# johanDDC/R-TuckER

Hardware: NVIDIA B200
Metric: train triples/s (1-N fwd+bwd+RSGD step), WN18RR (higher is better)
Workload: dtype f32 (score GEMMs and N x r x r passes: 3xTF32 on tcgen05 with round-to-nearest partial sums = fp32 accuracy, 1e-5 parity; Grams and N-independent stage f64)

## Files before the change

### r-tucker_b200/csrc/small.cu

```cuda
#include "small_kernels.cuh"
#include "small_exec.cuh"

#include <algorithm>
#include <vector>

namespace {
using namespace rt::small;
using rt::align_up;
using rt::cdiv;

constexpr int kNumT = 8;
constexpr int kMinDotSlots = 2048;
constexpr size_t kPartialArenaBytes = (size_t)592 * 64 * 64 * sizeof(double);

struct Layout {
  int r[3];
  int B;
  int64_t c;
  size_t C64, Gm[3], Ainv[3], coresq, Tn[kNumT], KC[3], Nn[3], Vf[3], GL[3], GLinv[3], Gs[3],
      tmpM[3], tmpK[3], sub[3], sub_shared, exec_bar, gemm_partial, gram_ws, dot_partial, scal, total;
  int dot_slots;
};

Layout make_layout(int r0, int r1, int r2, int B) {
// ... 253 lines not shown
           bool square_dev = false) {
    ew(EW_CVT, x, tx, n * dsize(tx), nullptr, 0, y, ty, n * dsize(ty), n, a_host, a_dev, 0.0, nullptr, square_dev ? 1 : 0);
  }
  void to32plain(const double* x, float* y, int64_t n) { cvt(x, DT_F64, y, DT_F32, n); }
  void scale32(const float* x, float* y, int64_t n, double a_host, const double* a_dev) { cvt(x, DT_F32, y, DT_F32, n, a_host, a_dev); }
  void to64(const float* x, double* y, int64_t n) { cvt(x, DT_F32, y, DT_F64, n); }
  void axpby(const double* x, const double* y, double* z, int64_t n, double a, const double* a_dev,
             double b, const double* b_dev) {
    ew(EW_AXPBY64, x, DT_F64, n * 8, y, n * 8, z, DT_F64, n * 8, n, a, a_dev, b, b_dev);
  }
  void copy2d(const void* src, int ts, int64_t lds, void* dst, int td, int64_t ldd, int rows, int cols) {
    ew(EW_CVT_2D, src, ts, ((size_t)(rows - 1) * lds + cols) * dsize(ts), nullptr, 0, dst, td,
       ((size_t)(rows - 1) * ldd + cols) * dsize(td), (int64_t)rows * cols, 1.0, nullptr, 0.0, nullptr, lds, ldd, rows, cols);
  }
  void transpose_into(const double* src, int n, double* dst, int64_t ldd) {
    ew(EW_TRANSPOSE_INTO, src, DT_F64, (size_t)n * n * 8, nullptr, 0, dst, DT_F64, ((size_t)(n - 1) * ldd + n) * 8,
       (int64_t)n * n, 1.0, nullptr, 0.0, nullptr, n, ldd, n, 0);
  }
  void symmetrize_lower(double* A, int n) {
    ew(EW_SYMM_LOWER, nullptr, DT_F64, 0, nullptr, 0, A, DT_F64, (size_t)n * n * 8, (int64_t)n * n, 1.0, nullptr, 0.0,
       nullptr, n, 0, n, 0, true);
  }
  void norm_finish(const double* sq, const double* hyper, double* norm_out, double* alpha_out) {
    if (err) return;
    Rec rec{};
    rec.op.kind = OP_EW; rec.op.ew = EW_NORM_FINISH; rec.op.units = 1;
    EwPart& e = rec.op.e;
    e.x = sq; e.y = alpha_out; e.z = norm_out; e.d0 = hyper; e.count = 1;
    rec.rd[rec.nrd++] = range(sq, 8);
    rec.rd[rec.nrd++] = range(hyper, 32);
    rec.wr[rec.nwr++] = range(norm_out, 8);
    rec.wr[rec.nwr++] = range(alpha_out, 8);
    push(rec);
  }
  void adam_finish(const double* sq, double* hyper, double* adam, double* norm_out, double* alpha_out) {
    if (err) return;
    Rec rec{};
    rec.op.kind = OP_EW; rec.op.ew = EW_ADAM_FINISH; rec.op.units = 1;
    EwPart& e = rec.op.e;
    e.x = sq; e.y = alpha_out; e.z = norm_out; e.d0 = hyper; e.d1 = adam; e.count = 1;
    rec.rd[rec.nrd++] = range(sq, 8);
    rec.rd[rec.nrd++] = range(adam, 64);
    rec.wr[rec.nwr++] = range(norm_out, 8);
    rec.wr[rec.nwr++] = range(alpha_out, 8);
    push(rec);
  }
  void zero64(double* z, int64_t n) { ew(EW_ZERO64, nullptr, DT_F64, 0, nullptr, 0, z, DT_F64, n * 8, n, 0.0, nullptr, 0.0, nullptr); }

  void dot(const void* x, int tx, const void* y, int ty, int64_t n, double scale, double* out, int accumulate) {
    if (err || n <= 0) return;
    const int64_t units64 = (n + kEwChunk - 1) / kEwChunk;
    if (units64 > L.dot_slots) {
      rt::set_error("small stage: a dot over %lld elements needs %lld partial slots, the workspace has %d",
                    (long long)n, (long long)units64, L.dot_slots);
      err = 2; return;
    }
    const int units = (int)units64;
    if (dot_off + units > L.dot_slots) { flush(); }
    double* part = p(L.dot_partial) + dot_off;
    dot_off += units;
    Rec rec{};
    rec.op.kind = OP_DOT;
    EwPart& e = rec.op.e;
    e.x = x; e.y = y; e.z = part; e.tx = tx; e.tz = ty; e.count = n;
    rec.op.units = units;
    rec.rd[rec.nrd++] = range(x, n * dsize(tx));
    rec.rd[rec.nrd++] = range(y, n * dsize(ty));
    rec.wr[rec.nwr++] = range(part, (size_t)units * 8);
    push(rec);
    Rec fin{};
    fin.op.kind = OP_DOTFIN;
    EwPart& f = fin.op.e;
    f.x = part; f.z = out; f.count = units; f.s0 = scale; f.p0 = accumulate;
    fin.op.units = 1;
    fin.rd[fin.nrd++] = range(part, (size_t)units * 8);
    if (accumulate) fin.rd[fin.nrd++] = range(out, 8);
    fin.wr[fin.nwr++] = range(out, 8);
    push(fin);
  }

  int spd(const SpdBatch& b, int count, int nmax) {
    flush();
    if (err) return 1;
    size_t smem = ((size_t)nmax * (nmax + 1) / 2 + (size_t)SPD_NB * nmax) * sizeof(double);
    const size_t smem_limit = 227 * 1024 - 3072;
    if (smem > smem_limit || nmax > 256) {
      rt::set_error("small stage: rank %d exceeds the in-shared-memory Cholesky limit (230)", nmax); return 2; }
    SpdBatch bb = b;
    bb.dmma = (smem + (size_t)SPD_NB * nmax * sizeof(double) <= smem_limit) ? 1 : 0;
    if (bb.dmma) smem += (size_t)SPD_NB * nmax * sizeof(double);
    if (cudaFuncSetAttribute(spd_blocked_kernel, cudaFuncAttributeMaxDynamicSharedMemorySize, (int)smem) != cudaSuccess) {
      rt::set_error("small stage: cannot raise shared memory to %zu", smem); return 1; }
    spd_blocked_kernel<<<count, SPD_THREADS, smem, s>>>(bb); ++rt::g_launches;
    return 0;
  }
};

int finish(Ctx& c, const char* what) {
  c.flush();
  if (c.err) { if (c.err == 1) rt::set_error("%s: kernel launch failed", what); return 1; }
  cudaError_t e = cudaGetLastError();
  if (e != cudaSuccess) { rt::set_error("%s: %s", what, cudaGetErrorString(e)); return 1; }
  return 0;
}

template <typename T>
void grouped_contract(Ctx& c, const T* X, const T* const B[3], const T* const Wa[3],
                      const T* const Wb[3], const int64_t st_o[3], const int64_t st_i[3],
                      T* D, T* E1, T* E2, T* U1, T* U2, T* out) {
  const int d[3] = {c.r(0), c.r(1), c.r(2)};
  c.mode_prod(0, Wa[0], st_o[0], st_i[0], d[0], d[0], X, d, D, 1.0, 0.0);
  c.mode_prod(0, Wb[0], st_o[0], st_i[0], d[0], d[0], B[0], d, D, 1.0, 1.0);
  c.mode_prod(0, Wa[0], st_o[0], st_i[0], d[0], d[0], B[1], d, E1, 1.0, 0.0);
  if (E2 != E1) c.mode_prod(0, Wa[0], st_o[0], st_i[0], d[0], d[0], B[2], d, E2, 1.0, 0.0);
  c.mode_prod(1, Wa[1], st_o[1], st_i[1], d[1], d[1], D, d, U1, 1.0, 0.0);
  c.mode_prod(1, Wb[1], st_o[1], st_i[1], d[1], d[1], E1, d, U1, 1.0, 1.0);
  c.mode_prod(1, Wa[1], st_o[1], st_i[1], d[1], d[1], E2, d, U2, 1.0, 0.0);
  c.mode_prod(2, Wa[2], st_o[2], st_i[2], d[2], d[2], U1, d, out, 1.0, 0.0);
  c.mode_prod(2, Wb[2], st_o[2], st_i[2], d[2], d[2], U2, d, out, 1.0, 1.0);
}

}

extern "C" size_t rt_small_ws_bytes(int r0, int r1, int r2, int B) {
  if (r0 <= 0 || r1 <= 0 || r2 <= 0) return 0;
  return make_layout(r0, r1, r2, B).total;
}

extern "C" int rt_small_prepare(const float* core, int r0, int r1, int r2, int sym, void* small_ws,
                                void* stream) {
  RT_REQUIRE(small_ws != nullptr && r0 > 0 && r1 > 0 && r2 > 0, "rt_small_prepare: bad arguments");
  RT_REQUIRE(!sym || r1 == r2, "rt_small_prepare: SF-Tucker needs r1 == r2");
  Ctx c{make_layout(r0, r1, r2, 0), (char*)small_ws, (cudaStream_t)stream};
  double* C64 = c.p(c.L.C64);
  c.to64(core, C64, c.L.c);
  const int d[3] = {r0, r1, r2};
  for (int i = 0; i < 3; ++i) c.unfold_gram(i, C64, d, C64, d[i], c.p(c.L.Gm[i]), d[i], 1.0, 0.0);
  if (sym) {
    c.axpby(c.p(c.L.Gm[1]), c.p(c.L.Gm[2]), c.p(c.L.Gm[1]), (int64_t)r1 * r1, 1.0, nullptr, 1.0, nullptr);
    c.axpby(c.p(c.L.Gm[1]), nullptr, c.p(c.L.Gm[2]), (int64_t)r1 * r1, 1.0, nullptr, 0.0, nullptr);
  }
  SpdBatch b{};
  int nmax = 0;
  for (int i = 0; i < 3; ++i) {
    b.p[i].G = c.p(c.L.Gm[i]); b.p[i].L = nullptr; b.p[i].Linv = nullptr; b.p[i].Ginv = c.p(c.L.Ainv[i]);
    b.p[i].n = d[i];
    nmax = d[i] > nmax ? d[i] : nmax;
  }
  c.dot(C64, DT_F64, C64, DT_F64, c.L.c, 1.0, c.p(c.L.coresq), 0);
  int rc = c.spd(b, 3, nmax);
  if (rc) return rc;
  return finish(c, "rt_small_prepare");
}

extern "C" size_t rt_small_ainv_offset(int mode, int r0, int r1, int r2) {
  if (mode < 0 || mode > 2) return (size_t)-1;
  return make_layout(r0, r1, r2, 0).Ainv[mode];
}

extern "C" int rt_rows_times_ainv(const float* A, int m, int mode, int r0, int r1, int r2, float* C,
                                  void* small_ws, void* stream) {
  RT_REQUIRE(mode >= 0 && mode < 3 && m >= 0, "rt_rows_times_ainv: bad arguments");
  if (m == 0) return 0;
  Layout L = make_layout(r0, r1, r2, 0);
  const int r = L.r[mode];
  const double* K = (const double*)((char*)small_ws + L.Ainv[mode]);
  const size_t smem = (size_t)4 * r * sizeof(float);
  rows_times_mat_kernel<<<cdiv(m, 4), 256, smem, (cudaStream_t)stream>>>(A, m, r, K, C);
  RT_LAUNCH_CHECK();
  return 0;
}

extern "C" int rt_small_grad(const float* core, const float* d_core, const float* qp, const float* H,
                             const float* r_rows, const float* s_rows, const float* dr_rows,
                             const float* ds_rows, const double* bce_sum, double inv_count,
                             const double* hyper, int B, int r0, int r1, int r2, int sym, float* dS_g,
// ... 211 lines not shown
```

### r-tucker_b200/csrc/small_kernels.cuh

```cuda
#pragma once
#include "common.h"
#include <math.h>

namespace rt {
namespace small {

__global__ void __launch_bounds__(256)
rows_times_mat_kernel(const float* __restrict__ A, int m, int r, const double* __restrict__ K,
                      float* __restrict__ C) {
  extern __shared__ float rows[];
  constexpr int RPB = 4;
  const int b0 = blockIdx.x * RPB;
  for (int e = threadIdx.x; e < RPB * r; e += 256) {
    const int rr = e / r, cc = e - rr * r;
    rows[e] = (b0 + rr < m) ? A[(int64_t)(b0 + rr) * r + cc] : 0.0f;
  }
  __syncthreads();
  for (int j = threadIdx.x; j < r; j += 256) {
    double acc[RPB];
#pragma unroll
    for (int i = 0; i < RPB; ++i) acc[i] = 0.0;
#pragma unroll 4
    for (int k = 0; k < r; ++k) {
      const double kv = K[(int64_t)k * r + j];
#pragma unroll
      for (int i = 0; i < RPB; ++i) acc[i] = fma((double)rows[i * r + k], kv, acc[i]);
    }
#pragma unroll
    for (int i = 0; i < RPB; ++i)
      if (b0 + i < m) C[(int64_t)(b0 + i) * r + j] = (float)acc[i];
  }
}

struct SpdProblem {
  const double* G;
  double* L;
  double* Linv;
  double* Ginv;
  int n;
};
struct SpdBatch { SpdProblem p[3]; int dmma; };

__device__ __forceinline__ int pk(int i, int j) { return i * (i + 1) / 2 + j; }
__device__ __forceinline__ void spd_dmma(double& c0, double& c1, double a, double b) {
  asm volatile("mma.sync.aligned.m8n8k4.row.col.f64.f64.f64.f64 {%0, %1}, {%2}, {%3}, {%0, %1};\n"
               : "+d"(c0), "+d"(c1) : "d"(a), "d"(b));
}
__device__ __forceinline__ double spd_sum8(const double (&c)[8][2], int e) {
  return ((c[0][e] + c[1][e]) + (c[2][e] + c[3][e])) + ((c[4][e] + c[5][e]) + (c[6][e] + c[7][e]));
}

constexpr int SPD_NB = 8;
constexpr int SPD_THREADS = 512, SPD_TPR = 2;
__global__ void __launch_bounds__(SPD_THREADS, 1)
spd_blocked_kernel(SpdBatch batch) {
  extern __shared__ double sm[];
  const SpdProblem P = batch.p[blockIdx.x];
  const int n = P.n;
  if (n <= 0) return;
  double* Lp = sm;
  double* stage = sm + n * (n + 1) / 2;
  __shared__ double D[SPD_NB][SPD_NB + 1], invd[SPD_NB];
  __shared__ double dinv_all[256];
  __shared__ double s_maxd, s_scale[4];
  const int tid = threadIdx.x, nt = blockDim.x;
  const int row = tid / SPD_TPR, sub = tid % SPD_TPR;
  for (int e = tid; e < n * (n + 1) / 2; e += nt) {
    int i = (int)((sqrt(8.0 * e + 1.0) - 1.0) * 0.5);
    while (i * (i + 1) / 2 > e) --i;
    while ((i + 1) * (i + 2) / 2 <= e) ++i;
    const int j = e - i * (i + 1) / 2;
    Lp[e] = 0.5 * (P.G[(int64_t)i * n + j] + P.G[(int64_t)j * n + i]);
  }
  __syncthreads();
  if (tid < 32) {
    double m = 0.0;
    for (int i = tid; i < n; i += 32) m = fmax(m, Lp[pk(i, i)]);
#pragma unroll
    for (int o = 16; o > 0; o >>= 1) m = fmax(m, __shfl_xor_sync(0xffffffffu, m, o));
    if (tid == 0) {
      int ex = 0;
      if (m > 0.0) { frexp(m, &ex); ex += ex & 1; }
      s_maxd = ldexp(m, -ex);
      s_scale[0] = ldexp(1.0, -ex);
      s_scale[1] = ldexp(1.0, ex / 2);
      s_scale[2] = ldexp(1.0, -(ex / 2));
      s_scale[3] = ldexp(1.0, -ex);
    }
  }
  __syncthreads();
  {
    const double sc = s_scale[0];
    for (int e = tid; e < n * (n + 1) / 2; e += nt) Lp[e] *= sc;
  }
  __syncthreads();
  const double tol = 1e-12 * s_maxd;
  double* Li = Lp + pk(row < n ? row : 0, 0);
#ifdef RT_SPD_PROF
  long long t_0 = clock64(), t_a = 0, t_b = 0, t_c = 0, t_x;
#define SPD_LAP(v) do { t_x = clock64(); v += t_x - t_0; t_0 = t_x; } while (0)
#else
#define SPD_LAP(v) do {} while (0)
#endif
  const bool use_dmma = batch.dmma != 0;
  const int warp = tid >> 5, lane = tid & 31, fg = lane >> 2, ft = lane & 3;
  constexpr int NW = SPD_THREADS / 32;
  double* accS = stage + SPD_NB * n;
  for (int kb = 0; kb < n; kb += SPD_NB) {
    const int nbk = min(SPD_NB, n - kb);
    if (use_dmma) {
      if (kb > 0) {
        const int ntile = (n - kb + 7) >> 3, nsteps = kb >> 2;
        const int brow = kb + fg;
        const bool bv = brow < n;
        const double* Lb = Lp + pk(bv ? brow : 0, 0) + ft;
        for (int tile = warp; tile < ntile; tile += NW) {
          const int arow = kb + 8 * tile + fg;
          const bool av = arow < n;
          const double* La = Lp + pk(av ? arow : 0, 0) + ft;
          double c[8][2];
#pragma unroll
          for (int u = 0; u < 8; ++u) { c[u][0] = 0.0; c[u][1] = 0.0; }
          for (int s0 = 0; s0 < nsteps; s0 += 8) {
#pragma unroll
            for (int u = 0; u < 8; ++u)
              if (s0 + u < nsteps) spd_dmma(c[u][0], c[u][1], av ? La[4 * (s0 + u)] : 0.0, bv ? Lb[4 * (s0 + u)] : 0.0);
          }
#pragma unroll
          for (int e = 0; e < 2; ++e) {
            const int col = 2 * ft + e;
            if (av && col < nbk && kb + col <= arow) Lp[pk(arow, kb + col)] -= spd_sum8(c, e);
          }
        }
      }
    } else {
      double acc[SPD_NB];
#pragma unroll
      for (int c = 0; c < SPD_NB; ++c) acc[c] = 0.0;
      if (row < n && row >= kb) {
        const double* Lc[SPD_NB];
#pragma unroll
        for (int c = 0; c < SPD_NB; ++c) Lc[c] = Lp + pk(kb + (c < nbk ? c : 0), 0);
        for (int k = sub; k < kb; k += SPD_TPR) {
          const double li = Li[k];
#pragma unroll
          for (int c = 0; c < SPD_NB; ++c) acc[c] = fma(li, Lc[c][k], acc[c]);
        }
      }
#pragma unroll
      for (int c = 0; c < SPD_NB; ++c) {
#pragma unroll
        for (int o = 1; o < SPD_TPR; o <<= 1) acc[c] += __shfl_xor_sync(0xffffffffu, acc[c], o);
      }
      if (row < n && row >= kb && sub == 0) {
#pragma unroll
        for (int c = 0; c < SPD_NB; ++c)
          if (c < nbk && kb + c <= row) Li[kb + c] -= acc[c];
      }
    }
    __syncthreads();
    SPD_LAP(t_a);
    if (tid < 32) {
      int er[2], ec[2];
#pragma unroll
      for (int u = 0; u < 2; ++u) {
        const int e = tid + 32 * u;
        int r = 0;
        while ((r + 1) * (r + 2) / 2 <= e) ++r;
        er[u] = r; ec[u] = e - r * (r + 1) / 2;
      }
      const bool has2 = tid + 32 < SPD_NB * (SPD_NB + 1) / 2;
      if (!has2) { er[1] = 0; ec[1] = 0; }
#pragma unroll
      for (int u = 0; u < 2; ++u)
        if (u == 0 || has2)
          D[er[u]][ec[u]] = (er[u] < nbk) ? Lp[pk(kb + er[u], kb + ec[u])] : (er[u] == ec[u] ? 1.0 : 0.0);
      __syncwarp();
#pragma unroll
      for (int c = 0; c < SPD_NB - 1; ++c) {
        const double dc = D[c][c];
        double a_rc[2], a_cc[2];
#pragma unroll
        for (int u = 0; u < 2; ++u) { a_rc[u] = D[er[u]][c]; a_cc[u] = D[ec[u]][c]; }
        double ri = 0.0;
        if (dc > tol) {
          double y = (double)__frcp_rn((float)dc);
          y = fma(y, fma(-dc, y, 1.0), y);
          ri = fma(y, fma(-dc, y, 1.0), y);
        }
#pragma unroll
        for (int u = 0; u < 2; ++u)
          if ((u == 0 || has2) && ec[u] > c) D[er[u]][ec[u]] = fma(-(a_rc[u] * a_cc[u]), ri, D[er[u]][ec[u]]);
        __syncwarp();
      }
      {
        const int c = tid & (SPD_NB - 1);
        const double dc = D[c][c];
        double piv = 0.0, inv = 0.0;
        if (dc > tol) {
          double y = (double)rsqrtf((float)dc);
#pragma unroll
          for (int it = 0; it < 2; ++it) y = y * fma(-0.5 * dc, y * y, 1.5);
          piv = dc * y;
          piv = fma(0.5 * y, fma(-piv, piv, dc), piv);
          inv = fma(y, fma(-piv, y, 1.0), y);
        }
        __syncwarp();
        if (tid < SPD_NB) {
          invd[c] = inv;
          if (c < nbk) dinv_all[kb + c] = inv;
        }
        __syncwarp();
#pragma unroll
        for (int u = 0; u < 2; ++u)
          if ((u == 0 || has2) && er[u] != ec[u]) D[er[u]][ec[u]] *= invd[ec[u]];
        if (tid < SPD_NB) D[c][c] = piv;
        __syncwarp();
#pragma unroll
        for (int u = 0; u < 2; ++u)
          if ((u == 0 || has2) && er[u] < nbk) Lp[pk(kb + er[u], kb + ec[u])] = D[er[u]][ec[u]];
      }
    }
    __syncthreads();
    SPD_LAP(t_b);
    if (row < n && row >= kb + nbk && sub == 0) {
      double xs[SPD_NB];
#pragma unroll
      for (int c = 0; c < SPD_NB; ++c) {
        if (c < nbk) {
          double x = Li[kb + c];
#pragma unroll
          for (int c2 = 0; c2 < SPD_NB; ++c2)
            if (c2 < c) x = fma(-xs[c2], D[c][c2], x);
          x *= invd[c];
          xs[c] = x;
          Li[kb + c] = x;
        }
      }
    }
    __syncthreads();
    SPD_LAP(t_c);
  }
#ifdef RT_SPD_PROF
  if (tid == 0) printf("spd n=%d chol: update %lld diag %lld panel %lld\n", n, t_a, t_b, t_c);
  t_a = t_b = t_c = 0; t_0 = clock64();
#endif
  if (P.L) {
    for (int e = tid; e < n * n; e += nt) {
      const int i = e / n, j = e - i * n;
      P.L[e] = (j <= i) ? Lp[pk(i, j)] * s_scale[1] : 0.0;
    }
  }
  if (!P.Linv && !P.Ginv) return;
  __syncthreads();
  for (int ib = 0; ib < n; ib += SPD_NB) {
    const int nbi = min(SPD_NB, n - ib);
    for (int e = tid; e < nbi * n; e += nt) {
      const int r = e / n, k = e - r * n;
      stage[e] = (k <= ib + r) ? Lp[pk(ib + r, k)] : 0.0;
    }
    __syncthreads();
    const int j = row;
    double acc[SPD_NB];
#pragma unroll
    for (int r = 0; r < SPD_NB; ++r) acc[r] = 0.0;
    if (use_dmma) {
      const int ntile = ib >> 3;
      for (int tile = warp; tile < ntile; tile += NW) {
        const int j0 = 8 * tile, jc = j0 + fg;
        const int nsteps = (ib - j0) >> 2;
        double c[8][2];
#pragma unroll
        for (int u = 0; u < 8; ++u) { c[u][0] = 0.0; c[u][1] = 0.0; }
        for (int s0 = 0; s0 < nsteps; s0 += 8) {
#pragma unroll
          for (int u = 0; u < 8; ++u)
            if (s0 + u < nsteps) {
              const int k = j0 + 4 * (s0 + u) + ft;
              spd_dmma(c[u][0], c[u][1], stage[fg * n + k], k >= jc ? Lp[pk(k, jc)] : 0.0);
            }
        }
#pragma unroll
        for (int e = 0; e < 2; ++e) accS[fg * n + j0 + 2 * ft + e] = spd_sum8(c, e);
      }
      __syncthreads();
      if (j < n && j < ib) {
#pragma unroll
        for (int r = 0; r < SPD_NB; ++r) acc[r] = accS[r * n + j];
      }
    } else {
      if (j < n && j < ib) {
        for (int k = j + sub; k < ib; k += SPD_TPR) {
          const double xk = Lp[pk(k, j)];
#pragma unroll
          for (int r = 0; r < SPD_NB; ++r) acc[r] = fma(stage[r * n + k], xk, acc[r]);
        }
      }
#pragma unroll
      for (int r = 0; r < SPD_NB; ++r) {
#pragma unroll
        for (int o = 1; o < SPD_TPR; o <<= 1) acc[r] += __shfl_xor_sync(0xffffffffu, acc[r], o);
      }
    }
    if (j < n && j < ib + nbi && sub == 0) {
      double xs[SPD_NB];
#pragma unroll
      for (int r = 0; r < SPD_NB; ++r) {
        xs[r] = 0.0;
        if (r < nbi) {
          const int i = ib + r;
          if (i >= j) {
            const double dinv = dinv_all[i];
            double x;
            if (i == j) {
              x = dinv;
            } else {
              double sacc = acc[r];
#pragma unroll
              for (int r2 = 0; r2 < SPD_NB; ++r2)
                if (r2 < r && ib + r2 >= j) sacc = fma(stage[r * n + ib + r2], xs[r2], sacc);
              x = -sacc * dinv;
            }
            xs[r] = x;
            Lp[pk(i, j)] = x;
          }
        }
      }
    }
    __syncthreads();
  }
  SPD_LAP(t_a);
  if (P.Linv) {
    for (int e = tid; e < n * n; e += nt) {
      const int i = e / n, j = e - i * n;
      P.Linv[e] = (j <= i) ? Lp[pk(i, j)] * s_scale[2] : 0.0;
    }
  }
  SPD_LAP(t_b);
  if (P.Ginv && use_dmma) {
    __syncthreads();
    const int T8 = (n + 7) >> 3;
    const double sc = s_scale[3];
    for (int u0 = warp; u0 < T8 * (T8 + 1) / 2; u0 += NW) {
      int it = (int)((sqrtf(8.0f * u0 + 1.0f) - 1.0f) * 0.5f);
      while (it * (it + 1) / 2 > u0) --it;
      while ((it + 1) * (it + 2) / 2 <= u0) ++it;
      const int jt = u0 - it * (it + 1) / 2;
      const int i0 = 8 * it, ic = i0 + fg, jc = 8 * jt + fg;
      const int nsteps = (n - i0 + 3) >> 2;
      double c[8][2];
#pragma unroll
      for (int u = 0; u < 8; ++u) { c[u][0] = 0.0; c[u][1] = 0.0; }
      for (int s0 = 0; s0 < nsteps; s0 += 8) {
#pragma unroll
        for (int u = 0; u < 8; ++u)
          if (s0 + u < nsteps) {
            const int k = i0 + 4 * (s0 + u) + ft;
            const bool kv = k < n;
            spd_dmma(c[u][0], c[u][1], (kv && ic < n && k >= ic) ? Lp[pk(k, ic)] : 0.0, (kv && jc < n && k >= jc) ? Lp[pk(k, jc)] : 0.0);
          }
      }
#pragma unroll
      for (int e = 0; e < 2; ++e) {
        const int i = i0 + fg, j = 8 * jt + 2 * ft + e;
        if (i < n && j <= i) {
          const double v = spd_sum8(c, e) * sc;
          P.Ginv[(int64_t)i * n + j] = v;
          P.Ginv[(int64_t)j * n + i] = v;
        }
      }
    }
  } else if (P.Ginv) {
    for (int e = tid; e < n * (n + 1) / 2; e += nt) {
      int i = (int)((sqrt(8.0 * e + 1.0) - 1.0) * 0.5);
      while (i * (i + 1) / 2 > e) --i;
      while ((i + 1) * (i + 2) / 2 <= e) ++i;
      const int j = e - i * (i + 1) / 2;
      double s0 = 0.0, s1 = 0.0, s2 = 0.0, s3 = 0.0;
      int k = i;
      for (; k + 3 < n; k += 4) {
        s0 = fma(Lp[pk(k, i)], Lp[pk(k, j)], s0);
        s1 = fma(Lp[pk(k + 1, i)], Lp[pk(k + 1, j)], s1);
        s2 = fma(Lp[pk(k + 2, i)], Lp[pk(k + 2, j)], s2);
        s3 = fma(Lp[pk(k + 3, i)], Lp[pk(k + 3, j)], s3);
      }
      for (; k < n; ++k) s0 = fma(Lp[pk(k, i)], Lp[pk(k, j)], s0);
      const double v = ((s0 + s1) + (s2 + s3)) * s_scale[3];
      P.Ginv[(int64_t)i * n + j] = v;
      P.Ginv[(int64_t)j * n + i] = v;
    }
  }
  SPD_LAP(t_c);
#ifdef RT_SPD_PROF
  if (tid == 0) printf("spd n=%d inverse %lld write Linv %lld Ginv %lld\n", n, t_a, t_b, t_c);
#endif
}

}
}
```

Measured before the change: 200,700.

## Distribute batched SPD Cholesky and inverse across 8-CTA thread-block clusters

Replaces the one-CTA-per-matrix packed-triangle Cholesky/inverse kernel with a cluster kernel. Each of 8 CTAs owns a round-robin set of 8-row block rows, and panel rows are broadcast to peers through distributed shared memory. The triangular inverse and Ginv products are likewise split by column blocks, with double-buffered staging overlapped with DMMA compute. This targets the serial small-rank factorisation on the N-independent stage, which used only three CTAs. In exchange it adds cluster synchronisation per block step, a residency check, and considerably more complex indexing.

```diff
diff --git a/r-tucker_b200/csrc/small.cu b/r-tucker_b200/csrc/small.cu
--- a/r-tucker_b200/csrc/small.cu
+++ b/r-tucker_b200/csrc/small.cu
@@ -359,16 +359,39 @@
   int spd(const SpdBatch& b, int count, int nmax) {
     flush();
     if (err) return 1;
-    size_t smem = ((size_t)nmax * (nmax + 1) / 2 + (size_t)SPD_NB * nmax) * sizeof(double);
-    const size_t smem_limit = 227 * 1024 - 3072;
-    if (smem > smem_limit || nmax > 256) {
-      rt::set_error("small stage: rank %d exceeds the in-shared-memory Cholesky limit (230)", nmax); return 2; }
-    SpdBatch bb = b;
-    bb.dmma = (smem + (size_t)SPD_NB * nmax * sizeof(double) <= smem_limit) ? 1 : 0;
-    if (bb.dmma) smem += (size_t)SPD_NB * nmax * sizeof(double);
-    if (cudaFuncSetAttribute(spd_blocked_kernel, cudaFuncAttributeMaxDynamicSharedMemorySize, (int)smem) != cudaSuccess) {
-      rt::set_error("small stage: cannot raise shared memory to %zu", smem); return 1; }
-    spd_blocked_kernel<<<count, SPD_THREADS, smem, s>>>(bb); ++rt::g_launches;
+    if (nmax > SPD_MAXN) {
+      rt::set_error("small stage: rank %d exceeds the SPD kernel's limit (%d)", nmax, SPD_MAXN); return 2; }
+    const size_t smem = spd_smem_bytes(nmax);
+    cudaLaunchConfig_t cfg = {};
+    cfg.gridDim = dim3(count * SPD_CLUSTER);
+    cfg.blockDim = dim3(SPD_THREADS);
+    cfg.dynamicSmemBytes = smem;
+    cfg.stream = s;
+    cudaLaunchAttribute attr[1];
+    attr[0].id = cudaLaunchAttributeClusterDimension;
+    attr[0].val.clusterDim.x = SPD_CLUSTER; attr[0].val.clusterDim.y = 1; attr[0].val.clusterDim.z = 1;
+    cfg.attrs = attr; cfg.numAttrs = 1;
+    constexpr int kDevs = 16;
+    static bool checked[kDevs];
+    int dev = 0;
+    cudaGetDevice(&dev);
+    if (dev >= kDevs || !checked[dev]) {
+      const size_t smem_max = spd_smem_bytes(SPD_MAXN);
+      cudaLaunchConfig_t probe = cfg;
+      probe.gridDim = dim3(3 * SPD_CLUSTER);
+      probe.dynamicSmemBytes = smem_max;
+      int clusters = 0;
+      if (rt::ensure_dyn_smem((const void*)spd_cluster_kernel, smem_max) != cudaSuccess ||
+          cudaOccupancyMaxActiveClusters(&clusters, spd_cluster_kernel, &probe) != cudaSuccess || clusters < 3) {
+        rt::set_error("small stage: cannot keep three %d-CTA clusters of %zu bytes of shared memory resident (%d)",
+                      SPD_CLUSTER, smem_max, clusters);
+        return 1;
+      }
+      if (dev < kDevs) checked[dev] = true;
+    }
+    const cudaError_t e = cudaLaunchKernelEx(&cfg, spd_cluster_kernel, b);
+    ++rt::g_launches;
+    if (e != cudaSuccess) { rt::set_error("small stage: SPD kernel launch: %s", cudaGetErrorString(e)); return 1; }
     return 0;
   }
 };
diff --git a/r-tucker_b200/csrc/small_kernels.cuh b/r-tucker_b200/csrc/small_kernels.cuh
--- a/r-tucker_b200/csrc/small_kernels.cuh
+++ b/r-tucker_b200/csrc/small_kernels.cuh
@@ -1,6 +1,8 @@
 #pragma once
 #include "common.h"
+#include <cooperative_groups.h>
 #include <math.h>
+#include <algorithm>
 
 namespace rt {
 namespace small {
@@ -39,9 +41,8 @@
   double* Ginv;
   int n;
 };
-struct SpdBatch { SpdProblem p[3]; int dmma; };
-
-__device__ __forceinline__ int pk(int i, int j) { return i * (i + 1) / 2 + j; }
+struct SpdBatch { SpdProblem p[3]; };
+
 __device__ __forceinline__ void spd_dmma(double& c0, double& c1, double a, double b) {
   asm volatile("mma.sync.aligned.m8n8k4.row.col.f64.f64.f64.f64 {%0, %1}, {%2}, {%3}, {%0, %1};\n"
                : "+d"(c0), "+d"(c1) : "d"(a), "d"(b));
@@ -50,32 +51,88 @@
   return ((c[0][e] + c[1][e]) + (c[2][e] + c[3][e])) + ((c[4][e] + c[5][e]) + (c[6][e] + c[7][e]));
 }
 
+template <typename SrcOff, typename DstOff>
+__device__ __forceinline__ void spd_copy4(int m, int t, int nthr, SrcOff so, DstOff dof, const double* src, double* dst) {
+  for (int e0 = t; e0 < m; e0 += 4 * nthr) {
+    double2 v[4];
+#pragma unroll
+    for (int u = 0; u < 4; ++u)
+      if (e0 + u * nthr < m) v[u] = *reinterpret_cast<const double2*>(src + so(e0 + u * nthr));
+#pragma unroll
+    for (int u = 0; u < 4; ++u)
+      if (e0 + u * nthr < m) *reinterpret_cast<double2*>(dst + dof(e0 + u * nthr)) = v[u];
+  }
+}
+
 constexpr int SPD_NB = 8;
-constexpr int SPD_THREADS = 512, SPD_TPR = 2;
+constexpr int SPD_MAXN = 256;
+constexpr int SPD_CLUSTER = 8;
+constexpr int SPD_THREADS = 512;
+constexpr int SPD_XLD = 12;
+constexpr int SPD_MAXOWN = (SPD_MAXN / SPD_NB + SPD_CLUSTER - 1) / SPD_CLUSTER;
+
+__host__ __device__ __forceinline__ int spd_nown(int rank, int T) {
+  return rank < T ? (T - rank + SPD_CLUSTER - 1) / SPD_CLUSTER : 0;
+}
+__host__ __device__ __forceinline__ int spd_rows_off(int rank, int lb) {
+  return 64 * (rank * lb + SPD_CLUSTER * (lb * (lb - 1) / 2)) + 96 * lb;
+}
+__host__ __device__ __forceinline__ int spd_cols_off(int rank, int lj, int T) {
+  return 8 * SPD_XLD * (T * lj - rank * lj - SPD_CLUSTER * (lj * (lj - 1) / 2));
+}
+__host__ __device__ __forceinline__ int spd_xchg_size(int T) {
+  return 16 * (8 * T + 4) > 16 * T * SPD_XLD ? 16 * (8 * T + 4) : 16 * T * SPD_XLD;
+}
+inline size_t spd_smem_bytes(int n) {
+  const int T = (n + SPD_NB - 1) / SPD_NB;
+  int own = 0;
+  for (int r = 0; r < SPD_CLUSTER; ++r) {
+    const int m = spd_nown(r, T);
+    own = std::max(own, spd_rows_off(r, m) + spd_cols_off(r, m, T));
+  }
+  return sizeof(double) * ((size_t)64 * T + spd_xchg_size(T) + own);
+}
+
 __global__ void __launch_bounds__(SPD_THREADS, 1)
-spd_blocked_kernel(SpdBatch batch) {
-  extern __shared__ double sm[];
-  const SpdProblem P = batch.p[blockIdx.x];
+spd_cluster_kernel(SpdBatch batch) {
+  namespace cg = cooperative_groups;
+  cg::cluster_group cluster = cg::this_cluster();
+  extern __shared__ __align__(16) double spd_sm[];
+  const SpdProblem P = batch.p[blockIdx.x / SPD_CLUSTER];
   const int n = P.n;
   if (n <= 0) return;
-  double* Lp = sm;
-  double* stage = sm + n * (n + 1) / 2;
+  constexpr int C = SPD_CLUSTER, NW = SPD_THREADS / 32;
+  const int R = (int)cluster.block_rank();
+  const int T = (n + 7) >> 3, SLD = 8 * T + 4;
+  const int nown = spd_nown(R, T);
+  double* Dg = spd_sm;
+  double* U = Dg + 64 * T;
+  double* rows = U + spd_xchg_size(T);
+  double* X = rows + spd_rows_off(R, nown);
   __shared__ double D[SPD_NB][SPD_NB + 1], invd[SPD_NB];
-  __shared__ double dinv_all[256];
+  __shared__ double dinv_all[SPD_MAXN];
+  __shared__ double accT[SPD_MAXOWN][SPD_NB][SPD_NB + 1];
   __shared__ double s_maxd, s_scale[4];
   const int tid = threadIdx.x, nt = blockDim.x;
-  const int row = tid / SPD_TPR, sub = tid % SPD_TPR;
-  for (int e = tid; e < n * (n + 1) / 2; e += nt) {
-    int i = (int)((sqrt(8.0 * e + 1.0) - 1.0) * 0.5);
-    while (i * (i + 1) / 2 > e) --i;
-    while ((i + 1) * (i + 2) / 2 <= e) ++i;
-    const int j = e - i * (i + 1) / 2;
-    Lp[e] = 0.5 * (P.G[(int64_t)i * n + j] + P.G[(int64_t)j * n + i]);
-  }
-  __syncthreads();
+  const int warp = tid >> 5, lane = tid & 31, fg = lane >> 2, ft = lane & 3;
+  const double* G = P.G;
+  auto sym = [&](int i, int j) { return 0.5 * (G[(int64_t)i * n + j] + G[(int64_t)j * n + i]); };
+#ifdef RT_SPD_PROF
+  long long t_0 = clock64(), t_set = 0, t_chol = 0, t_diag = 0, t_wait = 0, t_inv = 0, t_ginv = 0, t_x, t_k;
+#define SPD_LAP(v) do { t_x = clock64(); v += t_x - t_0; t_0 = t_x; } while (0)
+#define SPD_REPORT()                                                                                                   \
+  do {                                                                                                                 \
+    if (R == 0 && tid == 0)                                                                                            \
+      printf("spd n=%d cluster %d: setup %lld chol %lld (diag path %lld, cluster barriers %lld) inverse %lld Ginv %lld\n", \
+             n, C, t_set, t_chol, t_diag, t_wait, t_inv, t_ginv);                                                      \
+  } while (0)
+#else
+#define SPD_LAP(v) do {} while (0)
+#define SPD_REPORT() do {} while (0)
+#endif
   if (tid < 32) {
     double m = 0.0;
-    for (int i = tid; i < n; i += 32) m = fmax(m, Lp[pk(i, i)]);
+    for (int i = tid; i < n; i += 32) m = fmax(m, sym(i, i));
 #pragma unroll
     for (int o = 16; o > 0; o >>= 1) m = fmax(m, __shfl_xor_sync(0xffffffffu, m, o));
     if (tid == 0) {
@@ -91,76 +148,50 @@
   __syncthreads();
   {
     const double sc = s_scale[0];
-    for (int e = tid; e < n * (n + 1) / 2; e += nt) Lp[e] *= sc;
-  }
-  __syncthreads();
+    for (int e = tid; e < 64 * T; e += nt) {
+      const int b = e >> 6, i = 8 * b + ((e >> 3) & 7), j = 8 * b + (e & 7);
+      Dg[e] = (i < n && j <= i) ? sym(i, j) * sc : 0.0;
+    }
+    for (int lb = 0; lb < nown; ++lb) {
+      const int b = R + C * lb, ld = 8 * b + 12;
+      double* A = rows + spd_rows_off(R, lb);
+      for (int e = tid; e < 8 * ld; e += nt) {
+        const int i = 8 * b + e / ld, j = e % ld;
+        A[e] = (i < n && j <= i) ? sym(i, j) * sc : 0.0;
+      }
+    }
+    for (int e = tid; e < spd_cols_off(R, nown, T); e += nt) X[e] = 0.0;
+    for (int e = tid; e < spd_xchg_size(T); e += nt) U[e] = 0.0;
+  }
   const double tol = 1e-12 * s_maxd;
-  double* Li = Lp + pk(row < n ? row : 0, 0);
+  cluster.sync();
+  SPD_LAP(t_set);
+
+  for (int k = 0; k < T; ++k) {
+    const int kb = 8 * k, nbk = min(SPD_NB, n - kb);
+    const double* LR = U + (k & 1) * 8 * SLD;
+    const int nsteps = kb >> 2;
 #ifdef RT_SPD_PROF
-  long long t_0 = clock64(), t_a = 0, t_b = 0, t_c = 0, t_x;
-#define SPD_LAP(v) do { t_x = clock64(); v += t_x - t_0; t_0 = t_x; } while (0)
-#else
-#define SPD_LAP(v) do {} while (0)
+    t_k = clock64();
 #endif
-  const bool use_dmma = batch.dmma != 0;
-  const int warp = tid >> 5, lane = tid & 31, fg = lane >> 2, ft = lane & 3;
-  constexpr int NW = SPD_THREADS / 32;
-  double* accS = stage + SPD_NB * n;
-  for (int kb = 0; kb < n; kb += SPD_NB) {
-    const int nbk = min(SPD_NB, n - kb);
-    if (use_dmma) {
-      if (kb > 0) {
-        const int ntile = (n - kb + 7) >> 3, nsteps = kb >> 2;
-        const int brow = kb + fg;
-        const bool bv = brow < n;
-        const double* Lb = Lp + pk(bv ? brow : 0, 0) + ft;
-        for (int tile = warp; tile < ntile; tile += NW) {
-          const int arow = kb + 8 * tile + fg;
-          const bool av = arow < n;
-          const double* La = Lp + pk(av ? arow : 0, 0) + ft;
-          double c[8][2];
-#pragma unroll
-          for (int u = 0; u < 8; ++u) { c[u][0] = 0.0; c[u][1] = 0.0; }
-          for (int s0 = 0; s0 < nsteps; s0 += 8) {
-#pragma unroll
-            for (int u = 0; u < 8; ++u)
-              if (s0 + u < nsteps) spd_dmma(c[u][0], c[u][1], av ? La[4 * (s0 + u)] : 0.0, bv ? Lb[4 * (s0 + u)] : 0.0);
-          }
-#pragma unroll
-          for (int e = 0; e < 2; ++e) {
-            const int col = 2 * ft + e;
-            if (av && col < nbk && kb + col <= arow) Lp[pk(arow, kb + col)] -= spd_sum8(c, e);
-          }
-        }
-      }
-    } else {
-      double acc[SPD_NB];
-#pragma unroll
-      for (int c = 0; c < SPD_NB; ++c) acc[c] = 0.0;
-      if (row < n && row >= kb) {
-        const double* Lc[SPD_NB];
-#pragma unroll
-        for (int c = 0; c < SPD_NB; ++c) Lc[c] = Lp + pk(kb + (c < nbk ? c : 0), 0);
-        for (int k = sub; k < kb; k += SPD_TPR) {
-          const double li = Li[k];
-#pragma unroll
-          for (int c = 0; c < SPD_NB; ++c) acc[c] = fma(li, Lc[c][k], acc[c]);
-        }
-      }
-#pragma unroll
-      for (int c = 0; c < SPD_NB; ++c) {
-#pragma unroll
-        for (int o = 1; o < SPD_TPR; o <<= 1) acc[c] += __shfl_xor_sync(0xffffffffu, acc[c], o);
-      }
-      if (row < n && row >= kb && sub == 0) {
-#pragma unroll
-        for (int c = 0; c < SPD_NB; ++c)
-          if (c < nbk && kb + c <= row) Li[kb + c] -= acc[c];
-      }
-    }
-    __syncthreads();
-    SPD_LAP(t_a);
-    if (tid < 32) {
+    if (warp == 0) {
+      if (k > 0) {
+        const double* La = LR + fg * SLD + ft;
+        double c[8][2];
+#pragma unroll
+        for (int u = 0; u < 8; ++u) { c[u][0] = 0.0; c[u][1] = 0.0; }
+        for (int s0 = 0; s0 < nsteps; s0 += 8) {
+#pragma unroll
+          for (int u = 0; u < 8; ++u)
+            if (s0 + u < nsteps) spd_dmma(c[u][0], c[u][1], La[4 * (s0 + u)], La[4 * (s0 + u)]);
+        }
+#pragma unroll
+        for (int e = 0; e < 2; ++e) {
+          const int col = 2 * ft + e;
+          if (kb + fg < n && col < nbk && col <= fg) Dg[64 * k + 8 * fg + col] -= spd_sum8(c, e);
+        }
+        __syncwarp();
+      }
       int er[2], ec[2];
 #pragma unroll
       for (int u = 0; u < 2; ++u) {
@@ -171,10 +202,11 @@
       }
       const bool has2 = tid + 32 < SPD_NB * (SPD_NB + 1) / 2;
       if (!has2) { er[1] = 0; ec[1] = 0; }
+      double* Dk = Dg + 64 * k;
 #pragma unroll
       for (int u = 0; u < 2; ++u)
         if (u == 0 || has2)
-          D[er[u]][ec[u]] = (er[u] < nbk) ? Lp[pk(kb + er[u], kb + ec[u])] : (er[u] == ec[u] ? 1.0 : 0.0);
+          D[er[u]][ec[u]] = (er[u] < nbk) ? Dk[8 * er[u] + ec[u]] : (er[u] == ec[u] ? 1.0 : 0.0);
       __syncwarp();
 #pragma unroll
       for (int c = 0; c < SPD_NB - 1; ++c) {
@@ -216,185 +248,221 @@
           if ((u == 0 || has2) && er[u] != ec[u]) D[er[u]][ec[u]] *= invd[ec[u]];
         if (tid < SPD_NB) D[c][c] = piv;
         __syncwarp();
+        double* own = (k % C == R) ? rows + spd_rows_off(R, k / C) : nullptr;
 #pragma unroll
         for (int u = 0; u < 2; ++u)
-          if ((u == 0 || has2) && er[u] < nbk) Lp[pk(kb + er[u], kb + ec[u])] = D[er[u]][ec[u]];
-      }
-    }
-    __syncthreads();
-    SPD_LAP(t_b);
-    if (row < n && row >= kb + nbk && sub == 0) {
-      double xs[SPD_NB];
-#pragma unroll
-      for (int c = 0; c < SPD_NB; ++c) {
-        if (c < nbk) {
-          double x = Li[kb + c];
-#pragma unroll
-          for (int c2 = 0; c2 < SPD_NB; ++c2)
-            if (c2 < c) x = fma(-xs[c2], D[c][c2], x);
-          x *= invd[c];
-          xs[c] = x;
-          Li[kb + c] = x;
-        }
-      }
-    }
-    __syncthreads();
-    SPD_LAP(t_c);
-  }
+          if ((u == 0 || has2) && er[u] < nbk) {
+            Dk[8 * er[u] + ec[u]] = D[er[u]][ec[u]];
+            if (own) own[er[u] * (kb + 12) + kb + ec[u]] = D[er[u]][ec[u]];
+          }
+      }
 #ifdef RT_SPD_PROF
-  if (tid == 0) printf("spd n=%d chol: update %lld diag %lld panel %lld\n", n, t_a, t_b, t_c);
-  t_a = t_b = t_c = 0; t_0 = clock64();
+      t_diag += clock64() - t_k;
 #endif
-  if (P.L) {
-    for (int e = tid; e < n * n; e += nt) {
-      const int i = e / n, j = e - i * n;
-      P.L[e] = (j <= i) ? Lp[pk(i, j)] * s_scale[1] : 0.0;
-    }
-  }
-  if (!P.Linv && !P.Ginv) return;
-  __syncthreads();
-  for (int ib = 0; ib < n; ib += SPD_NB) {
-    const int nbi = min(SPD_NB, n - ib);
-    for (int e = tid; e < nbi * n; e += nt) {
-      const int r = e / n, k = e - r * n;
-      stage[e] = (k <= ib + r) ? Lp[pk(ib + r, k)] : 0.0;
-    }
-    __syncthreads();
-    const int j = row;
-    double acc[SPD_NB];
-#pragma unroll
-    for (int r = 0; r < SPD_NB; ++r) acc[r] = 0.0;
-    if (use_dmma) {
-      const int ntile = ib >> 3;
-      for (int tile = warp; tile < ntile; tile += NW) {
-        const int j0 = 8 * tile, jc = j0 + fg;
-        const int nsteps = (ib - j0) >> 2;
+    } else if (k > 0) {
+      const double* Lb = LR + fg * SLD + ft;
+      for (int lb = (k >= R ? (k - R) / C + 1 : 0) + warp - 1; lb < nown; lb += NW - 1) {
+        const int b = R + C * lb, ld = 8 * b + 12, arow = 8 * b + fg;
+        double* A = rows + spd_rows_off(R, lb);
+        const double* La = A + fg * ld + ft;
         double c[8][2];
 #pragma unroll
         for (int u = 0; u < 8; ++u) { c[u][0] = 0.0; c[u][1] = 0.0; }
         for (int s0 = 0; s0 < nsteps; s0 += 8) {
 #pragma unroll
           for (int u = 0; u < 8; ++u)
-            if (s0 + u < nsteps) {
-              const int k = j0 + 4 * (s0 + u) + ft;
-              spd_dmma(c[u][0], c[u][1], stage[fg * n + k], k >= jc ? Lp[pk(k, jc)] : 0.0);
+            if (s0 + u < nsteps) spd_dmma(c[u][0], c[u][1], La[4 * (s0 + u)], Lb[4 * (s0 + u)]);
+        }
+#pragma unroll
+        for (int e = 0; e < 2; ++e) {
+          const int col = 2 * ft + e;
+          if (arow < n && col < nbk) A[fg * ld + kb + col] -= spd_sum8(c, e);
+        }
+      }
+    }
+    __syncthreads();
+    if (tid < 8 * nown) {
+      const int lb = tid >> 3, r = tid & 7, b = R + C * lb, i = 8 * b + r;
+      if (b > k && i < n) {
+        double* Li = rows + spd_rows_off(R, lb) + r * (8 * b + 12);
+        double xs[SPD_NB];
+#pragma unroll
+        for (int c = 0; c < SPD_NB; ++c) {
+          if (c < nbk) {
+            double x = Li[kb + c];
+#pragma unroll
+            for (int c2 = 0; c2 < SPD_NB; ++c2)
+              if (c2 < c) x = fma(-xs[c2], D[c][c2], x);
+            x *= invd[c];
+            xs[c] = x;
+            Li[kb + c] = x;
+          }
+        }
+      }
+    }
+    if (k + 1 < T && (k + 1) % C == R) {
+      __syncthreads();
+      const int b = k + 1, ld = 8 * b + 12, w2 = 4 * b;
+      const double* src = rows + spd_rows_off(R, b / C);
+      for (int e = tid; e < C * 8 * w2; e += nt) {
+        const int dst = e / (8 * w2), rem = e - dst * 8 * w2, r = rem / w2, q = rem - r * w2;
+        double* buf = cluster.map_shared_rank(U, dst) + (b & 1) * 8 * SLD;
+        *reinterpret_cast<double2*>(buf + r * SLD + 2 * q) = *reinterpret_cast<const double2*>(src + r * ld + 2 * q);
+      }
+    }
+#ifdef RT_SPD_PROF
+    t_k = clock64();
+#endif
+    cluster.sync();
+#ifdef RT_SPD_PROF
+    t_wait += clock64() - t_k;
+#endif
+  }
+  SPD_LAP(t_chol);
+  if (P.L) {
+    const double sc = s_scale[1];
+    for (int lb = 0; lb < nown; ++lb) {
+      const int b = R + C * lb, ld = 8 * b + 12;
+      const double* A = rows + spd_rows_off(R, lb);
+      for (int e = tid; e < 8 * n; e += nt) {
+        const int r = e / n, j = e - r * n, i = 8 * b + r;
+        if (i < n) P.L[(int64_t)i * n + j] = (j <= i) ? A[r * ld + j] * sc : 0.0;
+      }
+    }
+  }
+  if (!P.Linv && !P.Ginv) {
+    SPD_LAP(t_inv);
+    SPD_REPORT();
+    return;
+  }
+
+  auto stage_row_block = [&](int ib, int t0) {
+    const int owner = ib % C, ld = 8 * ib + 12, w2 = 4 * (ib - R);
+    const double* src = cluster.map_shared_rank(rows, owner) + spd_rows_off(owner, ib / C) + 8 * R;
+    double* dst = U + (ib & 1) * 8 * SLD + 8 * R;
+    spd_copy4(8 * w2, tid - t0, nt - t0, [&](int e) { const int r = e / w2; return r * ld + 2 * (e - r * w2); },
+              [&](int e) { const int r = e / w2; return r * SLD + 2 * (e - r * w2); }, src, dst);
+  };
+  for (int ib = 0; ib < T && nown > 0; ++ib) {
+    const int nbi = min(SPD_NB, n - 8 * ib);
+    if (warp < nown) {
+      const int lj = warp, jb = R + C * lj;
+      if (jb < ib) {
+        const double* Sa = U + (ib & 1) * 8 * SLD + fg * SLD + 8 * jb + ft;
+        const double* Xb = X + spd_cols_off(R, lj, T) + ft * SPD_XLD + fg;
+        const int nsteps = 2 * (ib - jb);
+        double c[8][2];
+#pragma unroll
+        for (int u = 0; u < 8; ++u) { c[u][0] = 0.0; c[u][1] = 0.0; }
+        for (int s0 = 0; s0 < nsteps; s0 += 8) {
+#pragma unroll
+          for (int u = 0; u < 8; ++u)
+            if (s0 + u < nsteps) spd_dmma(c[u][0], c[u][1], Sa[4 * (s0 + u)], Xb[4 * (s0 + u) * SPD_XLD]);
+        }
+#pragma unroll
+        for (int e = 0; e < 2; ++e) accT[lj][fg][2 * ft + e] = spd_sum8(c, e);
+      }
+    } else if (ib + 1 < T && ib + 1 > R) {
+      stage_row_block(ib + 1, 32 * nown);
+    }
+    __syncthreads();
+    if (tid < 8 * nown) {
+      const int lj = tid >> 3, jj = tid & 7, jb = R + C * lj, j = 8 * jb + jj;
+      if (jb <= ib && j < n) {
+        double* Xj = X + spd_cols_off(R, lj, T) + jj;
+        const double* Lkk = Dg + 64 * ib;
+        double xs[SPD_NB];
+#pragma unroll
+        for (int r = 0; r < SPD_NB; ++r) {
+          xs[r] = 0.0;
+          if (r < nbi) {
+            const int i = 8 * ib + r;
+            if (i >= j) {
+              const double dinv = dinv_all[i];
+              double x;
+              if (i == j) {
+                x = dinv;
+              } else {
+                double sacc = jb < ib ? accT[lj][r][jj] : 0.0;
+#pragma unroll
+                for (int r2 = 0; r2 < SPD_NB; ++r2)
+                  if (r2 < r && 8 * ib + r2 >= j) sacc = fma(Lkk[8 * r + r2], xs[r2], sacc);
+                x = -sacc * dinv;
+              }
+              xs[r] = x;
+              Xj[(i - 8 * jb) * SPD_XLD] = x;
             }
-        }
-#pragma unroll
-        for (int e = 0; e < 2; ++e) accS[fg * n + j0 + 2 * ft + e] = spd_sum8(c, e);
-      }
-      __syncthreads();
-      if (j < n && j < ib) {
-#pragma unroll
-        for (int r = 0; r < SPD_NB; ++r) acc[r] = accS[r * n + j];
-      }
-    } else {
-      if (j < n && j < ib) {
-        for (int k = j + sub; k < ib; k += SPD_TPR) {
-          const double xk = Lp[pk(k, j)];
-#pragma unroll
-          for (int r = 0; r < SPD_NB; ++r) acc[r] = fma(stage[r * n + k], xk, acc[r]);
-        }
-      }
-#pragma unroll
-      for (int r = 0; r < SPD_NB; ++r) {
-#pragma unroll
-        for (int o = 1; o < SPD_TPR; o <<= 1) acc[r] += __shfl_xor_sync(0xffffffffu, acc[r], o);
-      }
-    }
-    if (j < n && j < ib + nbi && sub == 0) {
-      double xs[SPD_NB];
-#pragma unroll
-      for (int r = 0; r < SPD_NB; ++r) {
-        xs[r] = 0.0;
-        if (r < nbi) {
-          const int i = ib + r;
-          if (i >= j) {
-            const double dinv = dinv_all[i];
-            double x;
-            if (i == j) {
-              x = dinv;
-            } else {
-              double sacc = acc[r];
-#pragma unroll
-              for (int r2 = 0; r2 < SPD_NB; ++r2)
-                if (r2 < r && ib + r2 >= j) sacc = fma(stage[r * n + ib + r2], xs[r2], sacc);
-              x = -sacc * dinv;
-            }
-            xs[r] = x;
-            Lp[pk(i, j)] = x;
           }
         }
       }
     }
     __syncthreads();
   }
-  SPD_LAP(t_a);
   if (P.Linv) {
-    for (int e = tid; e < n * n; e += nt) {
-      const int i = e / n, j = e - i * n;
-      P.Linv[e] = (j <= i) ? Lp[pk(i, j)] * s_scale[2] : 0.0;
-    }
-  }
-  SPD_LAP(t_b);
-  if (P.Ginv && use_dmma) {
+    const double sc = s_scale[2];
+    for (int lj = 0; lj < nown; ++lj) {
+      const int jb = R + C * lj;
+      const double* Xj = X + spd_cols_off(R, lj, T);
+      for (int e = tid; e < 8 * n; e += nt) {
+        const int i = e >> 3, jj = e & 7, j = 8 * jb + jj;
+        if (j < n) P.Linv[(int64_t)i * n + j] = (i >= 8 * jb) ? Xj[(i - 8 * jb) * SPD_XLD + jj] * sc : 0.0;
+      }
+    }
+  }
+  cluster.sync();
+  SPD_LAP(t_inv);
+  if (!P.Ginv) {
+    SPD_REPORT();
+    return;
+  }
+
+  auto stage_col_block = [&](int jt, int t0) {
+    const int owner = jt % C, m = 4 * (8 * T - 8 * jt);
+    const double* src = cluster.map_shared_rank(rows, owner) + spd_rows_off(owner, spd_nown(owner, T)) +
+                        spd_cols_off(owner, jt / C, T);
+    double* dst = U + (jt & 1) * 8 * T * SPD_XLD;
+    auto off = [](int e) { return (e >> 2) * SPD_XLD + 2 * (e & 3); };
+    spd_copy4(m, tid - t0, nt - t0, off, off, src, dst);
+  };
+  if (nown > 0) stage_col_block(0, 0);
+  __syncthreads();
+  for (int jt = 0; jt < T && nown > 0; ++jt) {
+    if (warp < nown) {
+      const int lj = warp, it = R + C * lj;
+      if (it >= jt) {
+        const int i0 = 8 * it, nsteps = (n - i0 + 3) >> 2;
+        const double* Xa = X + spd_cols_off(R, lj, T) + ft * SPD_XLD + fg;
+        const double* Vb = U + (jt & 1) * 8 * T * SPD_XLD + (i0 - 8 * jt + ft) * SPD_XLD + fg;
+        double c[8][2];
+#pragma unroll
+        for (int u = 0; u < 8; ++u) { c[u][0] = 0.0; c[u][1] = 0.0; }
+        for (int s0 = 0; s0 < nsteps; s0 += 8) {
+#pragma unroll
+          for (int u = 0; u < 8; ++u)
+            if (s0 + u < nsteps) spd_dmma(c[u][0], c[u][1], Xa[4 * (s0 + u) * SPD_XLD], Vb[4 * (s0 + u) * SPD_XLD]);
+        }
+        const double sc = s_scale[3];
+#pragma unroll
+        for (int e = 0; e < 2; ++e) {
+          const int i = i0 + fg, j = 8 * jt + 2 * ft + e;
+          if (i < n && j <= i) {
+            const double v = spd_sum8(c, e) * sc;
+            P.Ginv[(int64_t)i * n + j] = v;
+            P.Ginv[(int64_t)j * n + i] = v;
+          }
+        }
+      }
+    } else if (jt + 1 < T) {
+      stage_col_block(jt + 1, 32 * nown);
+    }
     __syncthreads();
-    const int T8 = (n + 7) >> 3;
-    const double sc = s_scale[3];
-    for (int u0 = warp; u0 < T8 * (T8 + 1) / 2; u0 += NW) {
-      int it = (int)((sqrtf(8.0f * u0 + 1.0f) - 1.0f) * 0.5f);
-      while (it * (it + 1) / 2 > u0) --it;
-      while ((it + 1) * (it + 2) / 2 <= u0) ++it;
-      const int jt = u0 - it * (it + 1) / 2;
-      const int i0 = 8 * it, ic = i0 + fg, jc = 8 * jt + fg;
-      const int nsteps = (n - i0 + 3) >> 2;
-      double c[8][2];
-#pragma unroll
-      for (int u = 0; u < 8; ++u) { c[u][0] = 0.0; c[u][1] = 0.0; }
-      for (int s0 = 0; s0 < nsteps; s0 += 8) {
-#pragma unroll
-        for (int u = 0; u < 8; ++u)
-          if (s0 + u < nsteps) {
-            const int k = i0 + 4 * (s0 + u) + ft;
-            const bool kv = k < n;
-            spd_dmma(c[u][0], c[u][1], (kv && ic < n && k >= ic) ? Lp[pk(k, ic)] : 0.0, (kv && jc < n && k >= jc) ? Lp[pk(k, jc)] : 0.0);
-          }
-      }
-#pragma unroll
-      for (int e = 0; e < 2; ++e) {
-        const int i = i0 + fg, j = 8 * jt + 2 * ft + e;
-        if (i < n && j <= i) {
-          const double v = spd_sum8(c, e) * sc;
-          P.Ginv[(int64_t)i * n + j] = v;
-          P.Ginv[(int64_t)j * n + i] = v;
-        }
-      }
-    }
-  } else if (P.Ginv) {
-    for (int e = tid; e < n * (n + 1) / 2; e += nt) {
-      int i = (int)((sqrt(8.0 * e + 1.0) - 1.0) * 0.5);
-      while (i * (i + 1) / 2 > e) --i;
-      while ((i + 1) * (i + 2) / 2 <= e) ++i;
-      const int j = e - i * (i + 1) / 2;
-      double s0 = 0.0, s1 = 0.0, s2 = 0.0, s3 = 0.0;
-      int k = i;
-      for (; k + 3 < n; k += 4) {
-        s0 = fma(Lp[pk(k, i)], Lp[pk(k, j)], s0);
-        s1 = fma(Lp[pk(k + 1, i)], Lp[pk(k + 1, j)], s1);
-        s2 = fma(Lp[pk(k + 2, i)], Lp[pk(k + 2, j)], s2);
-        s3 = fma(Lp[pk(k + 3, i)], Lp[pk(k + 3, j)], s3);
-      }
-      for (; k < n; ++k) s0 = fma(Lp[pk(k, i)], Lp[pk(k, j)], s0);
-      const double v = ((s0 + s1) + (s2 + s3)) * s_scale[3];
-      P.Ginv[(int64_t)i * n + j] = v;
-      P.Ginv[(int64_t)j * n + i] = v;
-    }
-  }
-  SPD_LAP(t_c);
-#ifdef RT_SPD_PROF
-  if (tid == 0) printf("spd n=%d inverse %lld write Linv %lld Ginv %lld\n", n, t_a, t_b, t_c);
-#endif
-}
-
-}
-}
+  }
+  cluster.sync();
+  SPD_LAP(t_ginv);
+  SPD_REPORT();
+#undef SPD_REPORT
+#undef SPD_LAP
+}
+
+}
+}
```

Result: faster. 208,500 (median of 6 runs) (+3.9%).
